# ALVI-Labs/frankenstein

Measured on AMD Instinct MI355X. Metric: neural frames/sec (train fwd+bwd+AdamW, whole job), higher is better.
Workload: dtype bf16; 1 GPU; brainformer-small (6L d=384 6x64 heads, N=6144 tokens) + 2-block perceiver, L1 head; fwd+bwd+clip+AdamW; per_gpu_batch=32, global_batch=32, frames_T=600, electrodes=256, parallelism=dp1, weights=random-init (seed 42)

## Files before the change

frankenstein_amd/csrc/gemm.hip:

```cpp
#include <type_traits>

#include "fk_common.h"

namespace {

#ifndef FK_EPI_UNROLL
#define FK_EPI_UNROLL 1
#endif
#include "gemm_tile.h"

struct NtArgs {
  const void* A; const void* B; void* C;
  const void* bias; const void* res;
  int64_t lda, ldb, ldc, ldr, res_rows;
  int M, N, K, vec_epi;
  int mode;
  void* aux; int64_t ldaux;
  const float* rope_table; int64_t rope_bs; int rope_T, rope_off, rope_D, rope_cols;
  int rope_qcols; int64_t rope_qoff;
};

#ifndef FK_NT_STORES_GEMM
#define FK_NT_STORES_GEMM 1
#endif
// ... 421 lines not shown
  }
}

template <int N> FK_DEV void vm_wait_barrier() {
  asm volatile("s_waitcnt vmcnt(%0)\n\ts_barrier" ::"n"(N) : "memory");
}
constexpr int G4_LDS = 4 * 2 * TILE_BYTES;
static_assert(G4_LDS <= 160 * 1024, "LDS of a CU");
template <typename TO>
__global__ __launch_bounds__(NTHREADS, 1) void gemm_nt_glds4_kernel(NtArgs p) {
  using T = bf16_t;
  extern __shared__ __attribute__((aligned(16))) char smem[];
  const int tid = threadIdx.x, lane = tid & 63;
  const int wave = __builtin_amdgcn_readfirstlane(tid >> 6);
  const int wm = wave >> 1, wn = wave & 1, li = lane & 31, lh = lane >> 5;
  const int ntn = (p.N + BN - 1) / BN;
  const TileRange tr = tile_range(((p.M + BM - 1) / BM) * ntn);
  const int nbx = tr.nbx, t_end = tr.end;

  const T* srcA[4];
  const T* srcB[4];
  auto set_src = [&](int tile) {
    const int m0 = (tile / ntn) * BM, n0 = (tile % ntn) * BN;
#pragma unroll
    for (int j = 0; j < 4; ++j) {
      srcA[j] = dma_src(p.A, m0, p.M, p.lda, wave * 4 + j, lane);
      srcB[j] = dma_src(p.B, n0, p.N, p.ldb, wave * 4 + j, lane);
    }
  };
  auto stage = [&](int buf, int k0) __attribute__((always_inline)) {
    char* as = smem + buf * 2 * TILE_BYTES + wave * 4096;
#pragma unroll
    for (int j = 0; j < 4; ++j) {
      __builtin_amdgcn_global_load_lds((glb_void_t*)(srcA[j] + k0), (lds_void_t*)(as + j * 1024), 16, 0, 0);
      __builtin_amdgcn_global_load_lds((glb_void_t*)(srcB[j] + k0), (lds_void_t*)(as + TILE_BYTES + j * 1024), 16, 0, 0);
    }
  };
  const int nk = p.K / 64;
  auto head = [&]() __attribute__((always_inline)) {
    stage(0, 0);
    if (nk > 1) stage(1, 64);
    if (nk > 2) stage(2, 128);
  };
  int tile = tr.beg + tr.jb;
  if (tile < t_end) { set_src(tile); head(); }
  for (; tile < t_end; tile += nbx) {
    const int m0 = (tile / ntn) * BM, n0 = (tile % ntn) * BN;
    f32x16 acc[2][2];
#pragma unroll
    for (int i = 0; i < 2; ++i)
#pragma unroll
      for (int j = 0; j < 2; ++j)
#pragma unroll
        for (int r = 0; r < 16; ++r) acc[i][j][r] = 0.0f;
    for (int kt = 0; kt < nk; ++kt) {
      const int after = nk - 1 - kt;
      if (after >= 2) vm_wait_barrier<16>(); else if (after == 1) vm_wait_barrier<8>(); else vm_wait_barrier<0>();
      if (kt + 3 < nk) stage((kt + 3) & 3, (kt + 3) * 64);
      const char* as = smem + (kt & 3) * 2 * TILE_BYTES;
      const char* bs = as + TILE_BYTES;
#pragma unroll
      for (int s = 0; s < 4; ++s) {
        Frag<T> fa[2], fb[2];
#pragma unroll
        for (int i = 0; i < 2; ++i) nt_frag<T>(fa[i], as, wm * 64 + i * 32 + li, s, lh);
#pragma unroll
        for (int j = 0; j < 2; ++j) nt_frag<T>(fb[j], bs, wn * 64 + j * 32 + li, s, lh);
#pragma unroll
        for (int i = 0; i < 2; ++i)
#pragma unroll
          for (int j = 0; j < 2; ++j) mma32<T>(acc[i][j], fb[j], fa[i]);
      }
    }
    __syncthreads();
#pragma unroll
    for (int i = 0; i < 2; ++i) {
      f32x16 (&sub)[1][2] = *reinterpret_cast<f32x16 (*)[1][2]>(&acc[i][0]);
      nt_epilogue<T, TO, false, 1>(p, sub, smem + 3 * 2 * TILE_BYTES + wave * 8192, m0 + wm * 64 + i * 32, n0 + wn * 64, lane, false);
    }
    if (tile + nbx < t_end) { set_src(tile + nbx); head(); }
  }
}

template <typename TO, int BN_>
__global__ __launch_bounds__(512, 2) void gemm_nt_big_kernel(NtArgs p) {
  using T = bf16_t;
  constexpr int BM_ = 256, WCOLS = BN_ / 64, WROWS = 8 / WCOLS, WM = BM_ / WROWS, MT = WM / 32;
  constexpr int A_BYTES = BM_ * ROW_BYTES, B_BYTES = BN_ * ROW_BYTES, STAGE = A_BYTES + B_BYTES;
  constexpr int A_PER_WAVE = BM_ / 64, B_PER_WAVE = BN_ / 64;
  extern __shared__ __attribute__((aligned(16))) char smem[];
  const int tid = threadIdx.x, lane = tid & 63;
  const int wave = __builtin_amdgcn_readfirstlane(tid >> 6);
  const int wm = wave / WCOLS, wn = wave % WCOLS, li = lane & 31, lh = lane >> 5;
  const int ntn = (p.N + BN_ - 1) / BN_;
  const TileRange tr = tile_range(((p.M + BM_ - 1) / BM_) * ntn);
  const int nbx = tr.nbx, t_end = tr.end;

  static_assert(STAGE >= 8 * 8192, "the epilogue stages 8 waves x 8 KiB through the second stage buffer");
  const T* srcA[A_PER_WAVE];
  const T* srcB[B_PER_WAVE];
  auto set_src = [&](int tile) {
    const int m0 = (tile / ntn) * BM_, n0 = (tile % ntn) * BN_;
#pragma unroll
    for (int j = 0; j < A_PER_WAVE; ++j) srcA[j] = dma_src(p.A, m0, p.M, p.lda, wave * A_PER_WAVE + j, lane);
#pragma unroll
    for (int j = 0; j < B_PER_WAVE; ++j) srcB[j] = dma_src(p.B, n0, p.N, p.ldb, wave * B_PER_WAVE + j, lane);
  };
  auto stage = [&](int buf, int k0) {
    char* as = smem + buf * STAGE;
#pragma unroll
    for (int j = 0; j < A_PER_WAVE; ++j)
      __builtin_amdgcn_global_load_lds((glb_void_t*)(srcA[j] + k0), (lds_void_t*)(as + (wave * A_PER_WAVE + j) * 1024), 16, 0, 0);
#pragma unroll
    for (int j = 0; j < B_PER_WAVE; ++j)
      __builtin_amdgcn_global_load_lds((glb_void_t*)(srcB[j] + k0), (lds_void_t*)(as + A_BYTES + (wave * B_PER_WAVE + j) * 1024), 16, 0, 0);
  };
  const int nk = p.K / 64;
  int tile = tr.beg + tr.jb;
  if (tile < t_end) { set_src(tile); stage(0, 0); }
  for (; tile < t_end; tile += nbx) {
    const int m0 = (tile / ntn) * BM_, n0 = (tile % ntn) * BN_;
    f32x16 acc[MT][2];
#pragma unroll
    for (int i = 0; i < MT; ++i)
#pragma unroll
      for (int j = 0; j < 2; ++j)
#pragma unroll
        for (int r = 0; r < 16; ++r) acc[i][j][r] = 0.0f;
    __syncthreads();
    for (int kt = 0; kt < nk; ++kt) {
      if (kt + 1 < nk) stage((kt + 1) & 1, (kt + 1) * 64);
      const char* as = smem + (kt & 1) * STAGE;
      const char* bs = as + A_BYTES;
#pragma unroll
      for (int s = 0; s < 4; ++s) {
        Frag<T> fa[MT], fb[2];
#pragma unroll
        for (int i = 0; i < MT; ++i) nt_frag<T>(fa[i], as, wm * WM + i * 32 + li, s, lh);
#pragma unroll
        for (int j = 0; j < 2; ++j) nt_frag<T>(fb[j], bs, wn * 64 + j * 32 + li, s, lh);
#pragma unroll
        for (int i = 0; i < MT; ++i)
#pragma unroll
          for (int j = 0; j < 2; ++j) mma32<T>(acc[i][j], fb[j], fa[i]);
      }
      __syncthreads();
    }
#pragma unroll
    for (int i = 0; i < MT; ++i) {
      f32x16 (&sub)[1][2] = *reinterpret_cast<f32x16 (*)[1][2]>(&acc[i][0]);
      nt_epilogue<T, TO, true, 1>(p, sub, smem + STAGE + wave * 8192, m0 + wm * WM + i * 32, n0 + wn * 64, lane, false);
    }
    if (tile + nbx < t_end) { set_src(tile + nbx); stage(0, 0); }
  }
}

template <int BN_, int RB, int NS> struct Ring {
  static constexpr int BM_ = 256;
  static constexpr int STAGE = (BM_ + BN_) * RB, A_BYTES = BM_ * RB;
  static constexpr int IN_SLOT = STAGE / 8192 < 8 ? STAGE / 8192 : 8;
  static constexpr int LDS = NS * STAGE + (8 - IN_SLOT) * 8192;
  static constexpr int APW = BM_ * RB / 8192, BPW = BN_ * RB / 8192, PER = APW + BPW;
  static_assert(LDS <= 160 * 1024, "ring does not fit the LDS of a CU");
};

template <typename TO, int BN_, int RB, int NS, int EPI>
// ... 275 lines not shown
    if (part != 0) { if (++bkt == nk) { bkt = 0; btile += nbx; if (btile < t_end) set_b(btile); } }
  };
  issue_a(0, -1);
  issue_b(0, -1);
  issue_a(1, -1);
  int sa = 0, sb = 0;
  for (int tile = tr.beg + tr.jb; tile < t_end; tile += nbx) {
    const int m0 = (tile / ntn) * BM_, n0 = (tile % ntn) * BN_;
    const bool last_tile = tile + nbx >= t_end;
    f32x16 acc[NT6];
#pragma unroll
    for (int j = 0; j < NT6; ++j)
#pragma unroll
      for (int r = 0; r < 16; ++r) acc[j][r] = 0.0f;
    for (int kt = 0; kt < nk; ++kt) {
      if (last_tile && kt == nk - 1) vm_wait_barrier<0>(); else vm_wait_barrier<APW>();
      const int fill_a = sa == 0 ? 2 : sa - 1, fill_b = sb ^ 1;
      const char* as = aslot(sa);
      const char* bs = bslot(sb);
#ifndef FK_RING_PROBE_NOMMA
#pragma unroll
      for (int s = 0; s < 4; ++s) {
        Frag<T> fa, fb[NT6];
        nt_frag<T>(fa, as, wave * 32 + li, s, lh);
#pragma unroll
        for (int j = 0; j < NT6; ++j) nt_frag<T>(fb[j], bs, j * 32 + li, s, lh);
#pragma unroll
        for (int j = 0; j < NT6; ++j) mma32<T>(acc[j], fb[j], fa);
        __builtin_amdgcn_sched_barrier(0);
        if (s < 2) issue_b(fill_b, s); else issue_a(fill_a, s - 2);
        __builtin_amdgcn_sched_barrier(0);
      }
#else
      issue_b(fill_b, -1);
      issue_a(fill_a, -1);
#endif
      sa = sa == 2 ? 0 : sa + 1;
      sb ^= 1;
    }
    asm volatile("s_barrier" ::: "memory");
    char* stg = wave < 4 ? aslot(sa == 0 ? 2 : sa - 1) + wave * 8192
              : (wave < 7 ? bslot(sb ^ 1) + (wave - 4) * 8192 : smem + 3 * R192_A + 2 * R192_B);
#ifdef FK_RING_PROBE_NOEPI
    if (acc[0][0] == 123.456f) ((float*)p.C)[tid] = acc[NT6 - 1][3];
#else
#pragma unroll
    for (int c = 0; c < 3; ++c) {
      f32x16 (&sub)[1][2] = *reinterpret_cast<f32x16 (*)[1][2]>(&acc[2 * c]);
      if (EPI == 0 && p.res) nt_epilogue<T, TO, true, 1, true, EPI>(p, sub, stg, m0 + wave * 32, n0 + 64 * c, lane, false);
      else nt_epilogue<T, TO, true, 1, false, EPI>(p, sub, stg, m0 + wave * 32, n0 + 64 * c, lane, false);
    }
#endif
  }
}

static unsigned persistent_grid(int64_t nt) {
  static const int g = [] { const char* e = getenv("FK_NT_GRID_MULT"); const int v = e ? atoi(e) : 4; return v < 1 ? 1 : (v > 64 ? 64 : v); }();
  const int64_t cap = 256LL * g;
  return (unsigned)(nt < cap ? nt : cap);
}

enum NtRoute { NT_RING2, NT_RING192, NT_RING128, NT_BIG, NT_GLDS4, NT_GLDS, NT_STAGED };

template <typename F> static void with_epi(const NtArgs& p, F f) {
  if (p.mode == 1) f(std::integral_constant<int, 1>{});
  else if (p.mode == 2) f(std::integral_constant<int, 2>{});
  else if (p.rope_table) f(std::integral_constant<int, 3>{});
  else f(std::integral_constant<int, 0>{});
}

template <typename TO> static void launch_nt_route(NtRoute route, const NtArgs& p, int64_t M, int64_t N, hipStream_t s) {
  const int64_t nwg = fk_cdiv(M, BM) * fk_cdiv(N, BN);
  const dim3 grid((unsigned)nwg), block(NTHREADS), block8(512);
  auto tiles256 = [&](int bn) { return dim3(persistent_grid(fk_cdiv(M, 256) * fk_cdiv(N, bn))); };
  switch (route) {
    case NT_RING2:
      with_epi(p, [&](auto epi) { fk_launch_lds<gemm_nt_ring2_kernel<TO, decltype(epi)::value>>(tiles256(256), block8, R2_LDS, s, p); });
      break;
    case NT_RING192: fk_launch_lds<gemm_nt_ring192_kernel<TO, 0>>(tiles256(192), block8, R192_LDS, s, p); break;
    case NT_RING128:
      with_epi(p, [&](auto epi) { fk_launch_lds<gemm_nt_ring_kernel<TO, 128, 128, 3, decltype(epi)::value>>(tiles256(128), block8, Ring<128, 128, 3>::LDS, s, p); });
      break;
    case NT_BIG: fk_launch_lds<gemm_nt_big_kernel<TO, 256>>(tiles256(256), block8, 2 * (256 + 256) * ROW_BYTES, s, p); break;
    case NT_GLDS4: fk_launch_lds<gemm_nt_glds4_kernel<TO>>(grid, block, G4_LDS, s, p); break;
    case NT_GLDS:
      hipLaunchKernelGGL((gemm_nt_glds_kernel<TO>), dim3((unsigned)(nwg < 512 ? nwg : 512)), block, 4 * TILE_BYTES, s, p);
      break;
    case NT_STAGED: hipLaunchKernelGGL((gemm_nt_kernel<bf16_t, TO>), grid, block, 4 * TILE_BYTES, s, p); break;
  }
}

template <typename T> struct TNT;
template <> struct TNT<bf16_t> { static constexpr int BKM = 64, ROWB = 256, CHUNKS = 16, STEPS = 4; };
template <> struct TNT<float> { static constexpr int BKM = 32, ROWB = 512, CHUNKS = 32, STEPS = 2; };

FK_DEV int tn_off_bf16(int row, int bytecol) {
  const int g = bytecol >> 6;
  return row * 256 + (((g ^ (row & 3)) << 6) | (bytecol & 63));
}

template <typename T> FK_DEV void tn_frag(Frag<T>& f, const char* tile, int cb, int s, int lane);
template <> FK_DEV void tn_frag<bf16_t>(Frag<bf16_t>& f, const char* tile, int cb, int s, int lane) {
  const int g = lane >> 4, i = lane & 15, h = g >> 1;
  const int col = cb + 16 * (g & 1) + 4 * (i & 3);
#pragma unroll
  for (int t = 0; t < 2; ++t) {
    const int row = 16 * s + 8 * h + 4 * t + (i >> 2);
    bf16x4 v = lds_read_tr4(reinterpret_cast<const bf16_t*>(tile + tn_off_bf16(row, col * 2)));
#pragma unroll
    for (int e = 0; e < 4; ++e) f.v[4 * t + e] = v[e];
  }
}
template <> FK_DEV void tn_frag<float>(Frag<float>& f, const char* tile, int cb, int s, int lane) {
  const int h = lane >> 5, c = cb + (lane & 31);
#pragma unroll
  for (int e = 0; e < 8; ++e)
    f.v[e] = *reinterpret_cast<const float*>(tile + (16 * s + 8 * h + e) * 512 + c * 4);
}

struct TnArgs {
  const void* A; const void* B; float* C; float* ws;
  int64_t lda, ldb, ldc;
  int M, N1, N2, rows_per_split, nsplit, accumulate;
};

template <typename T>
__global__ __launch_bounds__(NTHREADS, 2) void gemm_tn_kernel(TnArgs p) {
  extern __shared__ __attribute__((aligned(16))) char smem[];
  constexpr int BKM = TNT<T>::BKM, ROWB = TNT<T>::ROWB, CHUNKS = TNT<T>::CHUNKS, STEPS = TNT<T>::STEPS;
  constexpr int VEC = KT<T>::VEC;
  constexpr int LOG_CH = (CHUNKS == 16) ? 4 : 5;
  const int tid = threadIdx.x, lane = tid & 63, wave = tid >> 6;
  const int wm = wave >> 1, wn = wave & 1, li = lane & 31, lh = lane >> 5;
  const int nt2 = (p.N2 + BN - 1) / BN, ntiles = ((p.N1 + BM - 1) / BM) * nt2;
  const unsigned L = xcd_remap(blockIdx.x, gridDim.x);
  const int split = (int)(L / ntiles), tile = (int)(L % ntiles);
  const int a0 = (tile / nt2) * BM, b0 = (tile % nt2) * BN;
  const int mbeg = split * p.rows_per_split;
  const int mend = min(p.M, mbeg + p.rows_per_split);
  const T* A = (const T*)p.A;
  const T* B = (const T*)p.B;

  f32x16 acc[2][2];
#pragma unroll
  for (int i = 0; i < 2; ++i)
#pragma unroll
    for (int j = 0; j < 2; ++j)
#pragma unroll
      for (int r = 0; r < 16; ++r) acc[i][j][r] = 0.0f;

  u32x4 ra[4], rb[4];
  auto gload = [&](int mrow0) {
#pragma unroll
    for (int i = 0; i < 4; ++i) {
      const int id = tid + NTHREADS * i, row = id >> LOG_CH, ch = id & (CHUNKS - 1);
      const int m = mrow0 + row, ca = a0 + ch * VEC, cb = b0 + ch * VEC;
      u32x4 z = {0u, 0u, 0u, 0u};
      ra[i] = (m < mend && ca < p.N1) ? *reinterpret_cast<const u32x4*>(A + (int64_t)m * p.lda + ca) : z;
      rb[i] = (m < mend && cb < p.N2) ? *reinterpret_cast<const u32x4*>(B + (int64_t)m * p.ldb + cb) : z;
    }
  };
  auto lds_off = [&](int row, int ch) -> int {
    if constexpr (sizeof(T) == 2) return tn_off_bf16(row, ch * 16);
    else return row * ROWB + ch * 16;
  };
  auto lstore = [&](int buf) {
    char* as = smem + buf * 2 * TILE_BYTES;
    char* bs = as + TILE_BYTES;
#pragma unroll
    for (int i = 0; i < 4; ++i) {
      const int id = tid + NTHREADS * i, row = id >> LOG_CH, ch = id & (CHUNKS - 1);
      *reinterpret_cast<u32x4*>(as + lds_off(row, ch)) = ra[i];
      *reinterpret_cast<u32x4*>(bs + lds_off(row, ch)) = rb[i];
    }
  };

  const int nk = (mend - mbeg + BKM - 1) / BKM;
  if (nk > 0) {
    gload(mbeg);
    lstore(0);
  }
  __syncthreads();
  for (int kt = 0; kt < nk; ++kt) {
    if (kt + 1 < nk) gload(mbeg + (kt + 1) * BKM);
    const char* as = smem + (kt & 1) * 2 * TILE_BYTES;
    const char* bs = as + TILE_BYTES;
#pragma unroll
    for (int s = 0; s < STEPS; ++s) {
      Frag<T> fa[2], fb[2];
#pragma unroll
      for (int i = 0; i < 2; ++i) tn_frag<T>(fa[i], as, wm * 64 + i * 32, s, lane);
#pragma unroll
      for (int j = 0; j < 2; ++j) tn_frag<T>(fb[j], bs, wn * 64 + j * 32, s, lane);
#pragma unroll
      for (int i = 0; i < 2; ++i)
#pragma unroll
        for (int j = 0; j < 2; ++j) mma32<T>(acc[i][j], fa[i], fb[j]);
    }
    if (kt + 1 < nk) lstore((kt + 1) & 1);
    __syncthreads();
  }

  float* out = (p.nsplit > 1) ? p.ws + (int64_t)split * p.N1 * p.N2 : p.C;
  const int64_t ldo = (p.nsplit > 1) ? p.N2 : p.ldc;
  const bool accum = (p.nsplit == 1) && p.accumulate;
#pragma unroll
  for (int j = 0; j < 2; ++j) {
    const int n = b0 + wn * 64 + j * 32 + li;
    if (n >= p.N2) continue;
#pragma unroll
    for (int i = 0; i < 2; ++i)
#pragma unroll
      for (int r = 0; r < 16; ++r) {
        const int m = a0 + wm * 64 + i * 32 + acc_row(r, lh);
        if (m >= p.N1) continue;
        float* dst = out + (int64_t)m * ldo + n;
        *dst = accum ? (*dst + acc[i][j][r]) : acc[i][j][r];
      }
  }
}

constexpr int TG_A = 384, TG_B = 128, TG_K = 32;
constexpr int TG_NS = 4;
constexpr int TG_A_ROW = TG_A * 2, TG_B_ROW = TG_B * 2;
constexpr int TG_A_BYTES = TG_K * TG_A_ROW, TG_B_BYTES = TG_K * TG_B_ROW, TG_STAGE = TG_A_BYTES + TG_B_BYTES;

template <int PITCH> FK_DEV int tg_off(int row, int bytecol) {
  return row * PITCH + (bytecol & ~255) + ((((bytecol >> 6) ^ row) & 3) << 6) + (bytecol & 63);
}
template <int OFF> FK_DEV bf16x4 tr_read(unsigned base) {
  s16x4 r;
  asm volatile("ds_read_b64_tr_b16 %0, %1 offset:%2" : "=v"(r) : "v"(base), "n"(OFF) : "memory");
  return __builtin_bit_cast(bf16x4, r);
}
template <int N> FK_DEV void lgkm_wait() {
  asm volatile("s_waitcnt lgkmcnt(%0)" ::"n"(N) : "memory");
  __builtin_amdgcn_sched_barrier(0);
}
template <int PITCH, int S> FK_DEV void tg_frag(Frag<bf16_t>& f, unsigned base) {
  const bf16x4 v0 = tr_read<(16 * S) * PITCH>(base), v1 = tr_read<(16 * S + 4) * PITCH>(base);
#pragma unroll
  for (int e = 0; e < 4; ++e) { f.v[e] = v0[e]; f.v[4 + e] = v1[e]; }
}
FK_DEV unsigned lds_addr(const char* p) {
  return (unsigned)(__UINTPTR_TYPE__)((__attribute__((address_space(3))) const char*)p);
}

template <int TB>
__global__ __launch_bounds__(512, 2) void gemm_tn_big_kernel(TnArgs p) {
  constexpr int B_ROW = TB == 128 ? 256 : 512, B_BYTES = TG_K * B_ROW, STAGE = TG_A_BYTES + B_BYTES, NJ = TB / 64, WB = TB / 2;
  using T = bf16_t;
  extern __shared__ __attribute__((aligned(16))) char smem[];
  const int tid = threadIdx.x, lane = tid & 63;
  const int wave = __builtin_amdgcn_readfirstlane(tid >> 6);
  const int wm = wave >> 1, wn = wave & 1, li = lane & 31, lh = lane >> 5;
  const int nt2 = p.N2 / TB, ntiles = (p.N1 / TG_A) * nt2;
  const unsigned L = xcd_remap(blockIdx.x, gridDim.x);
  const int split = (int)(L / ntiles), tile = (int)(L % ntiles);
  const int a0 = (tile / nt2) * TG_A, b0 = (tile % nt2) * TB;
  const int mbeg = split * p.rows_per_split;
  const int mend = min(p.M, mbeg + p.rows_per_split);
  const int nk = (mend - mbeg) / TG_K;

  constexpr int APW = TG_A_BYTES / 8192, BPW = B_BYTES / 8192, PER = APW + BPW;
  const T* srcA[APW];
  const T* srcB[BPW];
#pragma unroll
  for (int j = 0; j < APW; ++j) {
    const int o = (wave * APW + j) * 1024 + lane * 16, row = o / TG_A_ROW, bc = o % TG_A_ROW;
    const int sc = (bc & ~255) + ((((bc >> 6) ^ row) & 3) << 6) + (bc & 63);
    srcA[j] = (const T*)p.A + (int64_t)(mbeg + row) * p.lda + a0 + sc / 2;
  }
#pragma unroll
  for (int j = 0; j < BPW; ++j) {
    const int o = (wave * BPW + j) * 1024 + lane * 16, row = o / B_ROW, bc = o % B_ROW;
    int sc = (bc & ~255) + ((((bc >> 6) ^ row) & 3) << 6) + (bc & 63);
    if (sc >= TB * 2) sc = 0;
    srcB[j] = (const T*)p.B + (int64_t)(mbeg + row) * p.ldb + b0 + sc / 2;
  }
  const int64_t astep = (int64_t)TG_K * p.lda, bstep = (int64_t)TG_K * p.ldb;
  auto piece = [&](int buf, int j) __attribute__((always_inline)) {
    char* as = smem + buf * STAGE;
    if (j < APW) {
      __builtin_amdgcn_global_load_lds((glb_void_t*)srcA[j], (lds_void_t*)(as + (wave * APW + j) * 1024), 16, 0, 0);
      srcA[j] += astep;
    } else {
      __builtin_amdgcn_global_load_lds((glb_void_t*)srcB[j - APW], (lds_void_t*)(as + TG_A_BYTES + (wave * BPW + j - APW) * 1024), 16, 0, 0);
      srcB[j - APW] += bstep;
    }
  };

  unsigned fbase[3 + NJ];
  {
    const int g = lane >> 4, i = lane & 15, row = 8 * (g >> 1) + (i >> 2), dc = 16 * (g & 1) + 4 * (i & 3);
#pragma unroll
    for (int q = 0; q < 3; ++q) fbase[q] = lds_addr(smem) + tg_off<TG_A_ROW>(row, (wm * 96 + q * 32 + dc) * 2);
#pragma unroll
    for (int q = 0; q < NJ; ++q) fbase[3 + q] = lds_addr(smem) + TG_A_BYTES + tg_off<B_ROW>(row, (wn * WB + q * 32 + dc) * 2);
  }

  f32x16 acc[3][NJ];
// ... 314 lines not shown
  return launch_nt("fk_gemm_nt_rope", A, lda, B, ldb, C, ldc, M, N, K, bias, nullptr, 0, 0, dtype, dtype, 0, nullptr, 0, stream,
                   RopeSpec{table, table_bs, (int)T, (int)pos_off, (int)D, (int)rot_cols, (int)q_cols, q_table_off});
}

int fk_gemm_nt_swiglu(const void* A, int64_t lda, const void* W13, int64_t ldb, void* H13, int64_t ldh, void* G,
                      int64_t ldg, int64_t M, int64_t H, int64_t K, int dtype, void* stream) {
  FK_CHECK_ARG(H > 0 && H % 4 == 0, "fk_gemm_nt_swiglu: hidden size must be a multiple of 4");
  if (swiglu_takes_lane(M, H, K, lda, ldb, ldh, ldg, aligned16(A, W13, H13, G), dtype))
    return fk_mlp_up_fused_launch(A, lda, W13, ldb, H13, ldh, G, ldg, M, H, stream);
  return launch_nt("fk_gemm_nt_swiglu", A, lda, W13, ldb, H13, ldh, M, 2 * H, K, nullptr, nullptr, 0, 0, dtype, dtype, 1, G, ldg, stream);
}

int fk_gemm_nt_dswiglu(const void* dY, int64_t lda, const void* W2T, int64_t ldb, const void* H13, int64_t ldh, void* dH13,
                       int64_t lddh, int64_t M, int64_t H, int64_t K, int dtype, void* stream) {
  FK_CHECK_ARG(H > 0 && H % 8 == 0, "fk_gemm_nt_dswiglu: hidden size must be a multiple of 8");
  FK_CHECK_ARG(lddh % 8 == 0 && ((uintptr_t)dH13 & 15) == 0, "fk_gemm_nt_dswiglu: dH13 must be 16-byte aligned with an 8-element stride");
  return launch_nt("fk_gemm_nt_dswiglu", dY, lda, W2T, ldb, dH13, lddh, M, H, K, nullptr, nullptr, 0, 0, dtype, dtype, 2,
                   const_cast<void*>(H13), ldh, stream);
}

int fk_gemm_nt_route(int64_t M, int64_t N, int64_t K, int dtype, int vec_epi, int mode, int has_rope) {
  FK_CHECK_ARG(dtype == FK_F32 || dtype == FK_BF16, "fk_gemm_nt_route: bad dtype %d", dtype);
  FK_CHECK_ARG(M > 0 && N > 0 && K > 0 && mode >= 0 && mode <= 2, "fk_gemm_nt_route: bad problem M=%lld N=%lld K=%lld mode=%d", (long long)M, (long long)N, (long long)K, mode);
  if (dtype == FK_F32) return FK_NT_ROUTE_F32;
  return (int)nt_route(M, N, K, dtype, vec_epi != 0, mode, has_rope != 0);
}

int fk_gemm_nt_rope_route(int64_t M, int64_t N, int64_t K, int64_t lda, int64_t ldb, int64_t ldc, int has_bias, int64_t T, int64_t pos_off,
                          int64_t D, int64_t rot_cols, int64_t q_cols, int align_ok, int dtype) {
  FK_CHECK_ARG(dtype == FK_F32 || dtype == FK_BF16, "fk_gemm_nt_rope_route: bad dtype %d", dtype);
  FK_CHECK_ARG(M > 0 && N > 0 && K > 0, "fk_gemm_nt_rope_route: bad problem M=%lld N=%lld K=%lld", (long long)M, (long long)N, (long long)K);
  if (rope_takes_lane(M, N, K, lda, ldb, ldc, has_bias != 0, T, pos_off, D, rot_cols, q_cols, align_ok != 0, dtype)) return FK_NT_LANE;
  if (dtype == FK_F32) return FK_NT_ROUTE_F32;
  return (int)nt_route(M, N, K, dtype, N % 8 == 0 && ldc % 8 == 0 && align_ok != 0, 0, true);
}

int fk_gemm_nt_swiglu_route(int64_t M, int64_t H, int64_t K, int64_t lda, int64_t ldb, int64_t ldh, int64_t ldg, int align_ok, int dtype) {
  FK_CHECK_ARG(dtype == FK_F32 || dtype == FK_BF16, "fk_gemm_nt_swiglu_route: bad dtype %d", dtype);
  FK_CHECK_ARG(M > 0 && H > 0 && K > 0, "fk_gemm_nt_swiglu_route: bad problem M=%lld H=%lld K=%lld", (long long)M, (long long)H, (long long)K);
  if (swiglu_takes_lane(M, H, K, lda, ldb, ldh, ldg, align_ok != 0, dtype)) return FK_NT_LANE;
  if (dtype == FK_F32) return FK_NT_ROUTE_F32;
  return (int)nt_route(M, 2 * H, K, dtype, (2 * H) % 8 == 0 && ldh % 8 == 0 && align_ok != 0, 1, false);
}

static int tn_plan(int64_t M, int64_t N1, int64_t N2, int dtype, int* nsplit, int64_t* rows_per_split) {
  const bool big = tn_big_ok(M, N1, N2, dtype);
  const int bkm = dtype == FK_BF16 ? 64 : 32;
  const int ns = big ? tn_big_splits(M, N1, N2) : tn_splits(M, N1, N2, bkm);
  if (nsplit) *nsplit = ns;
  if (rows_per_split) *rows_per_split = fk_cdiv(fk_cdiv(M, ns), bkm) * bkm;
  return big ? tn_big_tb(N1, N2) : 0;
}

int fk_gemm_tn_route(int64_t M, int64_t N1, int64_t N2, int dtype, int* nsplit, int64_t* rows_per_split) {
  FK_CHECK_ARG(dtype == FK_F32 || dtype == FK_BF16, "fk_gemm_tn_route: bad dtype %d", dtype);
  FK_CHECK_ARG(M > 0 && N1 > 0 && N2 > 0, "fk_gemm_tn_route: empty problem");
  return tn_plan(M, N1, N2, dtype, nsplit, rows_per_split);
}

size_t fk_gemm_tn_workspace_bytes(int64_t M, int64_t N1, int64_t N2, int dtype) {
  int ns;
  tn_plan(M, N1, N2, dtype, &ns, nullptr);
  return ns > 1 ? (size_t)ns * N1 * N2 * sizeof(float) : 0;
}

static int launch_tn(const void* A, int64_t lda, const void* B, int64_t ldb, float* C, float* C1, int64_t ldc, int64_t M, int64_t N1,
                     int64_t N2, int accumulate, int dtype, void* workspace, size_t workspace_bytes, void* stream) {
  FK_CHECK_ARG(dtype == FK_F32 || dtype == FK_BF16, "fk_gemm_tn: bad dtype %d", dtype);
  const int vec = dtype == FK_BF16 ? 8 : 4;
  FK_CHECK_ARG(M > 0 && N1 > 0 && N2 > 0, "fk_gemm_tn: empty problem");
  FK_CHECK_ARG(M < (1LL << 31) && N1 < (1LL << 31) && N2 < (1LL << 31), "fk_gemm_tn: dims must fit int32");
  FK_CHECK_ARG(N1 % vec == 0 && N2 % vec == 0 && lda % vec == 0 && ldb % vec == 0,
               "fk_gemm_tn: N1/N2/lda/ldb must be multiples of %d (N1=%lld N2=%lld)", vec, (long long)N1, (long long)N2);
  FK_CHECK_ARG(((uintptr_t)A & 15) == 0 && ((uintptr_t)B & 15) == 0, "fk_gemm_tn: A/B must be 16-byte aligned");
  int ns;
  int64_t rps;
  const int tb = tn_plan(M, N1, N2, dtype, &ns, &rps);
  const bool big = tb != 0;
  const size_t need = ns > 1 ? (size_t)ns * N1 * N2 * sizeof(float) : 0;
  FK_CHECK_ARG(workspace_bytes >= need && (need == 0 || workspace), "fk_gemm_tn: workspace too small (%zu < %zu)", workspace_bytes, need);
  if (C1)
    FK_CHECK_ARG(ns > 1 && N1 % 8 == 0 && N2 % 4 == 0 && ldc % 4 == 0 && (((uintptr_t)C | (uintptr_t)C1 | (uintptr_t)workspace) & 15) == 0,
                 "fk_gemm_tn_swiglu: needs a split plan (see fk_gemm_tn_route), N1 %% 8 == 0, N2 %% 4 == 0 and 16-byte aligned destinations");
  TnArgs p{A, B, C, (float*)workspace, lda, ldb, ldc, (int)M, (int)N1, (int)N2, (int)rps, ns, accumulate};
  dim3 grid((unsigned)(fk_cdiv(N1, BM) * fk_cdiv(N2, BN) * ns)), block(NTHREADS);
  hipStream_t s = (hipStream_t)stream;
  if (big) {
    dim3 bgrid((unsigned)((N1 / TG_A) * (N2 / tb) * ns));
    if (tb == 192) {
      constexpr int LDS192 = TG_NS * (TG_A_BYTES + TG_K * 512);
      fk_launch_lds<gemm_tn_big_kernel<192>>(bgrid, dim3(512), LDS192, s, p);
    } else {
      fk_launch_lds<gemm_tn_big_kernel<128>>(bgrid, dim3(512), TG_NS * TG_STAGE, s, p);
    }
  } else if (dtype == FK_BF16) hipLaunchKernelGGL((gemm_tn_kernel<bf16_t>), grid, block, 4 * TILE_BYTES, s, p);
  else hipLaunchKernelGGL((gemm_tn_kernel<float>), grid, block, 4 * TILE_BYTES, s, p);
  FK_CHECK_LAUNCH("fk_gemm_tn");
  if (ns > 1) {
    const int64_t total = N1 * N2;
    if (N2 % 4 == 0 && ldc % 4 == 0 && (((uintptr_t)C | (uintptr_t)workspace) & 15) == 0) {
      int nb = (int)fk_cdiv(total / 4, 256);
      if (nb > 2048) nb = 2048;
      if (C1) hipLaunchKernelGGL(reduce_slabs4_kernel<true>, dim3(nb), dim3(256), 0, s, (const float*)workspace, C, C1, ldc, (int)N1, (int)N2, ns, accumulate);
      else hipLaunchKernelGGL(reduce_slabs4_kernel<false>, dim3(nb), dim3(256), 0, s, (const float*)workspace, C, C1, ldc, (int)N1, (int)N2, ns, accumulate);
    } else {
      int nb = (int)fk_cdiv(total, 256);
      if (nb > 2048) nb = 2048;
      hipLaunchKernelGGL(reduce_slabs_kernel, dim3(nb), dim3(256), 0, s, (const float*)workspace, C, ldc, (int)N1, (int)N2, ns, accumulate);
    }
    FK_CHECK_LAUNCH("fk_gemm_tn(reduce)");
  }
  return FK_OK;
}

int fk_gemm_tn(const void* A, int64_t lda, const void* B, int64_t ldb, float* C, int64_t ldc, int64_t M, int64_t N1,
               int64_t N2, int accumulate, int dtype, void* workspace, size_t workspace_bytes, void* stream) {
  return launch_tn(A, lda, B, ldb, C, nullptr, ldc, M, N1, N2, accumulate, dtype, workspace, workspace_bytes, stream);
}

int fk_gemm_tn_swiglu(const void* A, int64_t lda, const void* B, int64_t ldb, float* d_up, float* d_gate, int64_t ldc, int64_t M,
                      int64_t H, int64_t N2, int dtype, void* workspace, size_t workspace_bytes, void* stream) {
  FK_CHECK_ARG(d_up && d_gate && H > 0 && H % 4 == 0, "fk_gemm_tn_swiglu: needs both destinations and H %% 4 == 0");
  return launch_tn(A, lda, B, ldb, d_up, d_gate, ldc, M, 2 * H, N2, 1, dtype, workspace, workspace_bytes, stream);
}

size_t fk_colsum_workspace_bytes(int64_t rows, int64_t cols) { return (size_t)colsum_blocks(rows) * cols * sizeof(float); }

int fk_colsum(const void* X, int64_t ld, float* out, int64_t rows, int64_t cols, int accumulate, int dtype,
              void* workspace, size_t workspace_bytes, void* stream) {
  FK_CHECK_ARG(dtype == FK_F32 || dtype == FK_BF16, "fk_colsum: bad dtype %d", dtype);
  FK_CHECK_ARG(rows > 0 && cols > 0 && rows < (1LL << 31) && cols < (1LL << 31), "fk_colsum: bad shape");
  const int nb = colsum_blocks(rows);
  FK_CHECK_ARG(workspace && workspace_bytes >= (size_t)nb * cols * sizeof(float), "fk_colsum: workspace too small");
  const int rpb = (int)fk_cdiv(rows, nb);
  hipStream_t s = (hipStream_t)stream;
  const int vec = dtype == FK_BF16 ? 8 : 4;
  if (cols % vec == 0 && ld % vec == 0 && ((uintptr_t)X & 15) == 0) {
    dim3 grid((unsigned)fk_cdiv(fk_cdiv(cols, vec), 256), (unsigned)nb), block(256);
    if (dtype == FK_BF16) hipLaunchKernelGGL(colsum_partial_kernel<bf16_t>, grid, block, 0, s, (const bf16_t*)X, ld, (float*)workspace, (int)rows, (int)cols, rpb);
    else hipLaunchKernelGGL(colsum_partial_kernel<float>, grid, block, 0, s, (const float*)X, ld, (float*)workspace, (int)rows, (int)cols, rpb);
  } else {
    dim3 grid((unsigned)fk_cdiv(cols, 256), (unsigned)nb), block(256);
    if (dtype == FK_BF16) hipLaunchKernelGGL(colsum_partial_scalar_kernel<bf16_t>, grid, block, 0, s, (const bf16_t*)X, ld, (float*)workspace, (int)rows, (int)cols, rpb);
    else hipLaunchKernelGGL(colsum_partial_scalar_kernel<float>, grid, block, 0, s, (const float*)X, ld, (float*)workspace, (int)rows, (int)cols, rpb);
  }
  FK_CHECK_LAUNCH("fk_colsum(partial)");
  hipLaunchKernelGGL(colsum_final_kernel, dim3((unsigned)fk_cdiv(cols, 64)), dim3(256), 0, s, (const float*)workspace, out, (int)cols, nb, accumulate);
  FK_CHECK_LAUNCH("fk_colsum(final)");
  return FK_OK;
}

}
```

Measured before the change: 399,800 frames/s.

## Add one-shot small GEMM kernels for NT and split-K TN shapes

Adds a 64-row NT GEMM kernel with a six-stage global-to-LDS ring, used when the tile count is at most 256, so small problems spread across more workgroups. Also adds a TN kernel that loads the whole split-K panel into LDS and reduces the splits inside one workgroup. This removes the separate slab-reduction launch and its workspace traffic, and writes the swiglu interleaved output directly. An env var restores the old path, and the new kernels run one block per CU with large LDS.

```diff
diff --git a/frankenstein_amd/csrc/gemm.hip b/frankenstein_amd/csrc/gemm.hip
--- a/frankenstein_amd/csrc/gemm.hip
+++ b/frankenstein_amd/csrc/gemm.hip
@@ -527,6 +527,89 @@
   }
 }
 
+constexpr int G1_BM = 64, G1_NS = 6, G1_PER = 6;
+constexpr int G1_A_BYTES = G1_BM * ROW_BYTES, G1_STAGE = G1_A_BYTES + TILE_BYTES, G1_LDS = G1_NS * G1_STAGE;
+static_assert(G1_LDS <= 160 * 1024, "LDS of a CU");
+static_assert(G1_LDS >= 4 * 8192, "the epilogue stages 4 waves x 8 KiB through the ring");
+static_assert(G1_NS * G1_PER < 64, "vmcnt counts to 63");
+static_assert(G1_PER * NTHREADS / 64 * 1024 == G1_STAGE, "four waves request a whole stage");
+constexpr int T1_TILE = 32, T1_ROWB = T1_TILE * 2, T1_ROWS = 1024, T1_SPLIT_ROWS = 256, T1_PART = 4 * 16 * 64 * 4;
+constexpr int T1_LDS = T1_ROWS * 2 * T1_ROWB + T1_PART;
+static_assert(T1_LDS <= 160 * 1024, "LDS of a CU");
+static_assert(T1_SPLIT_ROWS / 16 * 2 < 64, "vmcnt counts to 63");
+
+enum SmallKind { SMALL_NT, SMALL_TN };
+static bool oneshot_form(SmallKind kind, int64_t M, int64_t N, int nsplit = 0, int64_t rows_per_split = 0) {
+  const char* e = getenv("FK_SMALL_GEMM_OLD");
+  if (e && atoi(e) != 0) return false;
+  if (kind == SMALL_NT) return fk_cdiv(M, G1_BM) * fk_cdiv(N, BN) <= 256;
+  return nsplit <= 4 && rows_per_split <= T1_SPLIT_ROWS && nsplit * rows_per_split <= T1_ROWS;
+}
+template <typename TO>
+__global__ __launch_bounds__(NTHREADS, 1) void gemm_nt_oneshot_kernel(NtArgs p) {
+  using T = bf16_t;
+  extern __shared__ __attribute__((aligned(16))) char smem[];
+  const int tid = threadIdx.x, lane = tid & 63;
+  const int wave = __builtin_amdgcn_readfirstlane(tid >> 6);
+  const int wm = wave >> 1, wn = wave & 1, li = lane & 31, lh = lane >> 5;
+  const int ntn = (p.N + BN - 1) / BN;
+  const unsigned L = xcd_remap(blockIdx.x, gridDim.x);
+  const int m0 = (int)(L / ntn) * G1_BM, n0 = (int)(L % ntn) * BN;
+
+  const T* srcA[2];
+  const T* srcB[4];
+#pragma unroll
+  for (int j = 0; j < 2; ++j) srcA[j] = dma_src(p.A, m0, p.M, p.lda, wave * 2 + j, lane);
+#pragma unroll
+  for (int j = 0; j < 4; ++j) srcB[j] = dma_src(p.B, n0, p.N, p.ldb, wave * 4 + j, lane);
+  auto stage = [&](int slot, int k0) __attribute__((always_inline)) {
+    char* as = smem + slot * G1_STAGE;
+    char* bs = as + G1_A_BYTES;
+#pragma unroll
+    for (int j = 0; j < 2; ++j)
+      __builtin_amdgcn_global_load_lds((glb_void_t*)(srcA[j] + k0), (lds_void_t*)(as + (wave * 2 + j) * 1024), 16, 0, 0);
+#pragma unroll
+    for (int j = 0; j < 4; ++j)
+      __builtin_amdgcn_global_load_lds((glb_void_t*)(srcB[j] + k0), (lds_void_t*)(bs + (wave * 4 + j) * 1024), 16, 0, 0);
+  };
+  const int nk = p.K / 64, nhead = min(nk, G1_NS);
+  for (int kt = 0; kt < nhead; ++kt) stage(kt, kt * 64);
+
+  f32x16 acc[1][2];
+#pragma unroll
+  for (int j = 0; j < 2; ++j)
+#pragma unroll
+    for (int r = 0; r < 16; ++r) acc[0][j][r] = 0.0f;
+  int slot = 0, prev = G1_NS - 1;
+  for (int kt = 0; kt < nk; ++kt) {
+    const int after = kt == 0 ? nhead - 1 : min(nk - 1 - kt, G1_NS - 2);
+    switch (after) {
+      case 5: vm_wait_barrier<5 * G1_PER>(); break;
+      case 4: vm_wait_barrier<4 * G1_PER>(); break;
+      case 3: vm_wait_barrier<3 * G1_PER>(); break;
+      case 2: vm_wait_barrier<2 * G1_PER>(); break;
+      case 1: vm_wait_barrier<1 * G1_PER>(); break;
+      default: vm_wait_barrier<0>(); break;
+    }
+    if (kt >= 1 && kt + G1_NS - 1 < nk) stage(prev, (kt + G1_NS - 1) * 64);
+    const char* as = smem + slot * G1_STAGE;
+    const char* bs = as + G1_A_BYTES;
+#pragma unroll
+    for (int s = 0; s < 4; ++s) {
+      Frag<T> fa, fb[2];
+      nt_frag<T>(fa, as, wm * 32 + li, s, lh);
+#pragma unroll
+      for (int j = 0; j < 2; ++j) nt_frag<T>(fb[j], bs, wn * 64 + j * 32 + li, s, lh);
+#pragma unroll
+      for (int j = 0; j < 2; ++j) mma32<T>(acc[0][j], fb[j], fa);
+    }
+    prev = slot;
+    slot = slot + 1 == G1_NS ? 0 : slot + 1;
+  }
+  __syncthreads();
+  nt_epilogue<T, TO, false, 1>(p, acc, smem + wave * 8192, m0 + wm * 32, n0 + wn * 64, lane, false);
+}
+
 template <typename TO, int BN_>
 __global__ __launch_bounds__(512, 2) void gemm_nt_big_kernel(NtArgs p) {
   using T = bf16_t;
@@ -968,7 +1051,10 @@
       with_epi(p, [&](auto epi) { fk_launch_lds<gemm_nt_ring_kernel<TO, 128, 128, 3, decltype(epi)::value>>(tiles256(128), block8, Ring<128, 128, 3>::LDS, s, p); });
       break;
     case NT_BIG: fk_launch_lds<gemm_nt_big_kernel<TO, 256>>(tiles256(256), block8, 2 * (256 + 256) * ROW_BYTES, s, p); break;
-    case NT_GLDS4: fk_launch_lds<gemm_nt_glds4_kernel<TO>>(grid, block, G4_LDS, s, p); break;
+    case NT_GLDS4:
+      if (oneshot_form(SMALL_NT, M, N)) fk_launch_lds<gemm_nt_oneshot_kernel<TO>>(dim3((unsigned)(fk_cdiv(M, G1_BM) * fk_cdiv(N, BN))), block, G1_LDS, s, p);
+      else fk_launch_lds<gemm_nt_glds4_kernel<TO>>(grid, block, G4_LDS, s, p);
+      break;
     case NT_GLDS:
       hipLaunchKernelGGL((gemm_nt_glds_kernel<TO>), dim3((unsigned)(nwg < 512 ? nwg : 512)), block, 4 * TILE_BYTES, s, p);
       break;
@@ -1008,6 +1094,7 @@
   const void* A; const void* B; float* C; float* ws;
   int64_t lda, ldb, ldc;
   int M, N1, N2, rows_per_split, nsplit, accumulate;
+  float* C1;
 };
 
 template <typename T>
@@ -1103,6 +1190,82 @@
         float* dst = out + (int64_t)m * ldo + n;
         *dst = accum ? (*dst + acc[i][j][r]) : acc[i][j][r];
       }
+  }
+}
+
+FK_DEV void tn1_frag(Frag<bf16_t>& f, const char* img, int s, int lane) {
+  const int g = lane >> 4, i = lane & 15, h = g >> 1;
+  const int col = 16 * (g & 1) + 4 * (i & 3);
+#pragma unroll
+  for (int t = 0; t < 2; ++t) {
+    const int row = 16 * s + 8 * h + 4 * t + (i >> 2);
+    bf16x4 v = lds_read_tr4(reinterpret_cast<const bf16_t*>(img + row * T1_ROWB + col * 2));
+#pragma unroll
+    for (int e = 0; e < 4; ++e) f.v[4 * t + e] = v[e];
+  }
+}
+template <int N> FK_DEV void vm_wait() { asm volatile("s_waitcnt vmcnt(%0)" ::"n"(N) : "memory"); }
+
+template <bool IL>
+__global__ __launch_bounds__(NTHREADS, 1) void gemm_tn_oneshot_kernel(TnArgs p) {
+  using T = bf16_t;
+  extern __shared__ __attribute__((aligned(16))) char smem[];
+  const int tid = threadIdx.x, lane = tid & 63;
+  const int wave = __builtin_amdgcn_readfirstlane(tid >> 6);
+  const int li = lane & 31, lh = lane >> 5;
+  const int nt2 = (p.N2 + T1_TILE - 1) / T1_TILE;
+  const int a0 = (int)(blockIdx.x / nt2) * T1_TILE, b0 = (int)(blockIdx.x % nt2) * T1_TILE;
+  const int mbeg = wave * p.rows_per_split, mend = min(p.M, mbeg + p.rows_per_split);
+  const int nk = (wave < p.nsplit && mend > mbeg) ? (mend - mbeg + 63) / 64 : 0;
+  char* ai = smem + wave * p.rows_per_split * 2 * T1_ROWB;
+  char* bi = ai + p.rows_per_split * T1_ROWB;
+
+  const int lr = lane >> 2, lc = (lane & 3) * 8;
+  const bool a_ok = a0 + lc < p.N1, b_ok = b0 + lc < p.N2;
+  const T* ap = (const T*)p.A + (int64_t)(mbeg + lr) * p.lda + (a0 + lc);
+  const T* bp = (const T*)p.B + (int64_t)(mbeg + lr) * p.ldb + (b0 + lc);
+  const u32x4 zero = {0u, 0u, 0u, 0u};
+  for (int j = 0; j < 4 * nk; ++j) {
+    const bool row_ok = mbeg + 16 * j + lr < mend;
+    char* ad = ai + j * 1024;
+    char* bd = bi + j * 1024;
+    if (row_ok && a_ok) __builtin_amdgcn_global_load_lds((glb_void_t*)(ap + (int64_t)16 * j * p.lda), (lds_void_t*)ad, 16, 0, 0);
+    else *reinterpret_cast<u32x4*>(ad + lane * 16) = zero;
+    if (row_ok && b_ok) __builtin_amdgcn_global_load_lds((glb_void_t*)(bp + (int64_t)16 * j * p.ldb), (lds_void_t*)bd, 16, 0, 0);
+    else *reinterpret_cast<u32x4*>(bd + lane * 16) = zero;
+  }
+  f32x16 part;
+#pragma unroll
+  for (int r = 0; r < 16; ++r) part[r] = 0.0f;
+  vm_wait<0>();
+  for (int kt = 0; kt < nk; ++kt) {
+#pragma unroll
+    for (int s = 0; s < 4; ++s) {
+      Frag<T> fa, fb;
+      tn1_frag(fa, ai + kt * 64 * T1_ROWB, s, lane);
+      tn1_frag(fb, bi + kt * 64 * T1_ROWB, s, lane);
+      mma32<T>(part, fa, fb);
+    }
+  }
+  float* ps = reinterpret_cast<float*>(smem + p.nsplit * p.rows_per_split * 2 * T1_ROWB);
+  if (wave < p.nsplit) {
+#pragma unroll
+    for (int r = 0; r < 16; ++r) ps[(wave * 16 + r) * 64 + lane] = part[r];
+  }
+  __syncthreads();
+  const int n = b0 + li;
+#pragma unroll
+  for (int q = 0; q < 4; ++q) {
+    const int r = 4 * wave + q, m = a0 + acc_row(r, lh);
+    float s = ps[r * 64 + lane];
+    if (p.nsplit > 1) s = 0.0f + s;
+    for (int i = 1; i < p.nsplit; ++i) s += ps[(i * 16 + r) * 64 + lane];
+    if (m < p.N1 && n < p.N2) {
+      float* dst;
+      if constexpr (IL) dst = ((m & 4) ? p.C1 : p.C) + (int64_t)((m >> 3) * 4 + (m & 3)) * p.ldc + n;
+      else dst = p.C + (int64_t)m * p.ldc + n;
+      *dst = p.accumulate ? (*dst + s) : s;
+    }
   }
 }
 
@@ -1583,9 +1746,16 @@
   if (C1)
     FK_CHECK_ARG(ns > 1 && N1 % 8 == 0 && N2 % 4 == 0 && ldc % 4 == 0 && (((uintptr_t)C | (uintptr_t)C1 | (uintptr_t)workspace) & 15) == 0,
                  "fk_gemm_tn_swiglu: needs a split plan (see fk_gemm_tn_route), N1 %% 8 == 0, N2 %% 4 == 0 and 16-byte aligned destinations");
-  TnArgs p{A, B, C, (float*)workspace, lda, ldb, ldc, (int)M, (int)N1, (int)N2, (int)rps, ns, accumulate};
+  TnArgs p{A, B, C, (float*)workspace, lda, ldb, ldc, (int)M, (int)N1, (int)N2, (int)rps, ns, accumulate, C1};
   dim3 grid((unsigned)(fk_cdiv(N1, BM) * fk_cdiv(N2, BN) * ns)), block(NTHREADS);
   hipStream_t s = (hipStream_t)stream;
+  if (!big && dtype == FK_BF16 && oneshot_form(SMALL_TN, N1, N2, ns, rps)) {
+    const dim3 ogrid((unsigned)(fk_cdiv(N1, T1_TILE) * fk_cdiv(N2, T1_TILE)));
+    if (C1) fk_launch_lds<gemm_tn_oneshot_kernel<true>>(ogrid, block, T1_LDS, s, p);
+    else fk_launch_lds<gemm_tn_oneshot_kernel<false>>(ogrid, block, T1_LDS, s, p);
+    FK_CHECK_LAUNCH("fk_gemm_tn");
+    return FK_OK;
+  }
   if (big) {
     dim3 bgrid((unsigned)((N1 / TG_A) * (N2 / tb) * ns));
     if (tb == 192) {
```

Measured after the change: 401,400 frames/s, median of 6. About the same (+0.4%).
